# vniclas/VFM-Registration

Measured on AMD Instinct MI355X. Metric: registrations/sec (20k<->200k pts, 384-D), higher is better.
Workload: dtype fp6 (MX e2m3) coarse pass (scaled MFMA, fp32 scores + bounds from measured residuals) + int8 rescan (exact integer scores) + f32 refinement + f64 exact decision / f64 RANSAC

## Files before the change

### vfm-registration_amd/csrc/config.cpp

```cpp
#include "common.h"
#include "config.h"

#include <string.h>

#include <new>

struct vfm_config {
    VfmConfig c;
};

static const VfmConfig k_factory{};
static thread_local const VfmConfig* t_bound = nullptr;

const VfmConfig& vfm_cfg() { return t_bound ? *t_bound : k_factory; }

namespace {
struct Field {
    const char* name;
    int VfmConfig::*p;
};
const Field k_fields[] = {
    {"coarse_slices", &VfmConfig::force_slices},     {"match_stats", &VfmConfig::match_stats},
    {"i8_min_queries", &VfmConfig::i8_min_queries},  {"prep_grid", &VfmConfig::prep_grid},
    {"ransac_exact_only", &VfmConfig::ransac_exact_only}, {"ransac_fused", &VfmConfig::ransac_fused},
    {"coarse_qsets", &VfmConfig::coarse_qsets},      {"seed_units", &VfmConfig::seed_units},
    {"select_variant", &VfmConfig::select_variant},  {"mx6_t4", &VfmConfig::mx6_t4},
    {"mx6_tune", &VfmConfig::mx6_tune},
    {"mx6_ns3", &VfmConfig::mx6_ns3},                {"prep_form", &VfmConfig::prep_stream},
    {"finish_short", &VfmConfig::finish_short},      {"rescan_rows", &VfmConfig::rescan_rows},
    {"half_noi8", &VfmConfig::half_noi8},
    {"vit_preprocess_patch", &VfmConfig::vit_preprocess_patch}, {"vit_xcd", &VfmConfig::vit_xcd},
    {"vit_cfg_narrow", &VfmConfig::vit_cfg_narrow},  {"vit_cfg_wide", &VfmConfig::vit_cfg_wide},
    {"vit_wpw", &VfmConfig::vit_wpw},                {"vit_hot_a", &VfmConfig::vit_hot_a},
    {"vit_wide_tile", &VfmConfig::vit_wide_tile},    {"vit_lds_shape", &VfmConfig::vit_lds_shape},
    {"vit_att_lds_min", &VfmConfig::vit_att_lds_min}, {"vit_lds_min_wg", &VfmConfig::vit_lds_min_wg},
    {"vit_astat_min", &VfmConfig::vit_astat_min},    {"vit_astat_two", &VfmConfig::vit_astat_two},
    {"vit_astat_nw", &VfmConfig::vit_astat_nw},      {"vit_fused_qkv", &VfmConfig::vit_fused_qkv},
    {"vit_trace_fused", &VfmConfig::vit_trace_fused},  {"vit_fused_mlp", &VfmConfig::vit_fused_mlp},
    {"voxel_replay2", &VfmConfig::voxel_replay2},    {"voxel_one_launch", &VfmConfig::voxel_small},
    {"voxel_trace", &VfmConfig::voxel_trace},        {"voxel_grid_ppt", &VfmConfig::voxel_grid_ppt},
};

void set_coarse_variant(VfmConfig& c, int v) {
    if (v == 60 || v == 61) { c.rescan_rows = v == 61 ? 1 : 0; return; }
    if (v == 50 || v == 51) { c.finish_short = v == 51 ? 1 : 0; return; }
    if (v >= 40 && v <= 44) { c.prep_stream = v == 44 ? 4 : v == 43 ? 3 : v == 41 ? 1 : 0; return; }
    if (v == 32 || v == 33) { c.mx6_ns3 = v == 33 ? 1 : 0; return; }
    if (v == 30 || v == 31) { c.mx6_t4 = v == 30 ? 1 : 0; return; }
    c.seed_units = v == 7 ? 0 : 1;
    if (v == 7) v = 0;
    c.select_variant = v == 20 ? 1 : (v == 21 ? 2 : 0);
    if (v == 20 || v == 21) v = 0;
    c.coarse_qsets = v;
}
void set_vit_gemm(VfmConfig& c, int narrow, int wide) {
    switch (narrow) {
        case -3: case -4: c.vit_xcd = narrow == -3 ? 1 : 0; return;
        case -5: c.vit_lds_min_wg = wide; return;
        case -6: c.vit_lds_shape = wide; return;
        case -7: c.vit_att_lds_min = wide; return;
        case -8: c.vit_wpw = wide; return;
        case -9: c.vit_astat_min = wide; return;
        case -10: c.vit_astat_nw = wide; return;
        case -11: case -12: {
            unsigned long long v = (unsigned long long)(uintptr_t)c.vit_astat_dbg;
            v = narrow == -11 ? ((v & 0xffffffff00000000ull) | (unsigned)wide) : ((v & 0xffffffffull) | ((unsigned long long)(unsigned)wide << 32));
            c.vit_astat_dbg = reinterpret_cast<unsigned long long*>((uintptr_t)v);
            return;
        }
        case -14: c.vit_preprocess_patch = wide; return;
        case -15: c.vit_astat_two = wide; return;
        case -16: c.vit_hot_a = wide; return;
        case -17: c.vit_wide_tile = wide; return;
        default:
            c.vit_cfg_narrow = narrow ? narrow : 108;
            c.vit_cfg_wide = wide ? wide : 108;
    }
}
void set_voxel_small(VfmConfig& c, int on) {
    if (on == 2 || on == 3) c.voxel_replay2 = on == 3;
    else if (on >= 10 && on <= 10 + 64) c.voxel_grid_ppt = on - 10;
    else if (on == 100 || on == 101) c.voxel_trace = on - 100;
    else c.voxel_small = on;
}
}

VFM_EXPORT int vfm_config_create(vfm_config_t** out) {
    VFM_CHECK_ARG(out, "config_create: null pointer");
    *out = new (std::nothrow) vfm_config();
    if (!*out) return vfm_fail(VFM_EINVAL, "config_create: out of memory");
    return VFM_OK;
}
VFM_EXPORT int vfm_config_destroy(vfm_config_t* cfg) {
    if (cfg && t_bound == &cfg->c) t_bound = nullptr;
    delete cfg;
    return VFM_OK;
}
VFM_EXPORT int vfm_config_use(const vfm_config_t* cfg) {
    t_bound = cfg ? &cfg->c : nullptr;
    return VFM_OK;
}
VFM_EXPORT int vfm_config_set(vfm_config_t* cfg, const char* key, int64_t value) {
    VFM_CHECK_ARG(cfg && key, "config_set: null pointer");
    if ((!strcmp(key, "coarse_variant") && value == 42) || (!strcmp(key, "prep_form") && value == 2))
        return vfm_fail(VFM_EINVAL, "config_set: %s %lld (fp6 operand preparation by width) has been removed", key, (long long)value);
    if (!strcmp(key, "coarse_variant")) { set_coarse_variant(cfg->c, (int)value); return VFM_OK; }
    if (!strcmp(key, "voxel_small")) { set_voxel_small(cfg->c, (int)value); return VFM_OK; }
    if (!strcmp(key, "vit_gemm")) { set_vit_gemm(cfg->c, (int)(value >> 32), (int)(int32_t)(uint32_t)(value & 0xffffffffll)); return VFM_OK; }
    for (const Field& f : k_fields)
        if (!strcmp(key, f.name)) {
            cfg->c.*(f.p) = (int)value;
            return VFM_OK;
        }
    return vfm_fail(VFM_EINVAL, "config_set: unknown key '%s'", key);
}
VFM_EXPORT int vfm_config_get(const vfm_config_t* cfg, const char* key, int64_t* value) {
    VFM_CHECK_ARG(key && value, "config_get: null pointer");
    const VfmConfig& c = cfg ? cfg->c : vfm_cfg();
    for (const Field& f : k_fields)
        if (!strcmp(key, f.name)) {
            *value = c.*(f.p);
            return VFM_OK;
        }
    return vfm_fail(VFM_EINVAL, "config_get: unknown key '%s'", key);
}
```

### vfm-registration_amd/csrc/config.h

```cpp
#pragma once

struct VfmConfig {
    int force_slices = 0;
    int coarse_qsets = 0;
    int seed_units = 1;
    int select_variant = 0;
    int mx6_t4 = 1;
    int mx6_ns3 = 1;
    int prep_stream = 3;
    int finish_short = 0;
    int half_noi8 = 1;
    int rescan_rows = 1;
    int mx6_tune = 0;
    int match_stats = 0;
    int i8_min_queries = 0;
    int prep_grid = -1;
    int ransac_exact_only = 0;
    int ransac_fused = 2;
    int vit_preprocess_patch = 1, vit_xcd = 1, vit_cfg_narrow = 108, vit_cfg_wide = 108, vit_wpw = 0, vit_hot_a = 0, vit_wide_tile = 0,
        vit_lds_shape = 23, vit_att_lds_min = 1, vit_lds_min_wg = 256, vit_astat_min = 0, vit_astat_two = 1, vit_astat_nw = 0,
        vit_trace_fused = 0,
        vit_fused_mlp = 0,
        vit_fused_qkv = 0;
    unsigned long long* vit_astat_dbg = nullptr;
    int voxel_replay2 = 1, voxel_small = 1, voxel_trace = 0, voxel_grid_ppt = 0;
};

const VfmConfig& vfm_cfg();
```

### vfm-registration_amd/csrc/match_finish.hip

```cpp
#include "match_internal.h"

namespace vfmm {
namespace {

constexpr int SELECT_GROUPS = 16;
__global__ __launch_bounds__(64 * SELECT_GROUPS) void match_select_kernel(const uint2* __restrict__ partials, int nchunks, int npad,
                                                           int64_t n, int first_pad_chunk,
                                                           const unsigned* __restrict__ qmax,
                                                           const float* __restrict__ invq, float window,
                                                           I8Bounds ib, float gate, int chunk_lds, int* __restrict__ cand_cnt,
                                                           unsigned* __restrict__ cand, int cap, int* __restrict__ fb_count,
                                                           int* __restrict__ fb_list, int stats) {
    extern __shared__ __attribute__((aligned(16))) unsigned char select_smem[];
    __shared__ int lcnt[64];
    __shared__ int lresc[64];
    __shared__ unsigned lub[64];
    const int qq = threadIdx.x & 63, g = threadIdx.x >> 6;
    const int64_t q = (int64_t)blockIdx.x * 64 + qq;
    if (g == 0) {
        lcnt[qq] = 0;
        lresc[qq] = 0;
        lub[qq] = 0u;
    }
    float2* lchunk = reinterpret_cast<float2*>(select_smem);
// ... 1258 lines not shown
__global__ __launch_bounds__(256) void match_rescan_kernel(int64_t n, int64_t m, int d, I8Bounds ib, const uint4* __restrict__ q8,
                                                           const uint4* __restrict__ b8, const unsigned* __restrict__ qmax,
                                                           int* __restrict__ cand_cnt, unsigned* __restrict__ cand, int cap,
                                                           unsigned* __restrict__ hits, int hcap, int* __restrict__ fb_count,
                                                           int* __restrict__ fb_list, int use_gate, float gate,
                                                           const int* __restrict__ guard, L2Terms l2) {
    __shared__ uint4 l_q8[4][48];
    const int lane = lane_id(), wave = threadIdx.x >> 6;
    const int64_t qi = (int64_t)blockIdx.x * 4 + wave;
    if (qi >= n) return;
    if (guard && *guard) {
        if (lane == 0) cand_cnt[qi] = 0;
        return;
    }
    const int cnt = cand_cnt[qi];
    if (cnt <= 0) return;
    if (cnt > cap) {
        if (lane == 0) {
            cand_cnt[qi] = -1;
            fb_list[atomicAdd(fb_count, 1)] = (int)qi;
        }
        return;
    }
    unsigned* mycand = cand + (size_t)qi * cap;
    unsigned* myhits = hits + (size_t)qi * hcap;
    const int units8 = d >> 4;
    if (lane < units8) l_q8[wave][lane] = q8[(size_t)(qi >> 5) * (units8 * 32) + (size_t)lane * 32 + (qi & 31)];
    const float eq = ib.qerr[qi];
    const float sq = ib.qstep[qi >> 7], A = eq * 1.0001220703125f + 1.0e-6f, mult = 1.0001220703125f + eq;
    const float qlow = use_gate ? gate : key_float(qmax[qi]);
    const float qn_l2 = l2.qn ? l2.qn[qi] : 0.0f;
    __builtin_amdgcn_wave_barrier();
    int nhit = 0;
    const bool direct = cnt <= 64;
    unsigned* out = direct ? mycand : myhits;
    const int ocap = direct ? cap : hcap;
    for (int e0 = 0; e0 < cnt; e0 += 64) {
        const unsigned batch = (e0 + lane < cnt) ? mycand[e0 + lane] : 0u;
        const int nb = cnt - e0 < 64 ? cnt - e0 : 64;
        for (int j = 0; j < nb; ++j) {
            const unsigned entry = __shfl(batch, j);
            const int c = (int)(entry >> 8);
            if (!(entry & 128u)) {
                if (lane == 0 && nhit < ocap) out[nhit] = entry;
                ++nhit;
                continue;
            }
            const long long base = (long long)c * CHUNK_ROWS;
            const float sc = sq * ib.bstep[c], bound = A + mult * ib.berr[c];
            const uint4* src0 = b8 + ((size_t)c * 4 + (lane >> 5)) * (size_t)(units8 * 32) + (lane & 31);
            const uint4* src1 = src0 + 2 * (size_t)(units8 * 32);
            int acc2[2] = {0, 0};
            for (int u0 = 0; u0 < units8; u0 += 8) {
                uint4 bv0[8], bv1[8];
#pragma unroll
                for (int k = 0; k < 8; ++k) {
                    bv0[k] = src0[(u0 + k) * 32];
                    bv1[k] = src1[(u0 + k) * 32];
                }
#pragma unroll
                for (int k = 0; k < 8; ++k) {
                    const uint4 qv = l_q8[wave][u0 + k];
                    acc2[0] = __builtin_amdgcn_sdot4((int)bv0[k].x, (int)qv.x, acc2[0], false);
                    acc2[0] = __builtin_amdgcn_sdot4((int)bv0[k].y, (int)qv.y, acc2[0], false);
                    acc2[0] = __builtin_amdgcn_sdot4((int)bv0[k].z, (int)qv.z, acc2[0], false);
                    acc2[0] = __builtin_amdgcn_sdot4((int)bv0[k].w, (int)qv.w, acc2[0], false);
                    acc2[1] = __builtin_amdgcn_sdot4((int)bv1[k].x, (int)qv.x, acc2[1], false);
                    acc2[1] = __builtin_amdgcn_sdot4((int)bv1[k].y, (int)qv.y, acc2[1], false);
                    acc2[1] = __builtin_amdgcn_sdot4((int)bv1[k].z, (int)qv.z, acc2[1], false);
                    acc2[1] = __builtin_amdgcn_sdot4((int)bv1[k].w, (int)qv.w, acc2[1], false);
                }
            }
#pragma unroll
            for (int half = 0; half < 2; ++half) {
                const int rr = lane + 64 * half;
                const int acc = acc2[half];
                float up = sc * (float)acc + bound;
                if (l2.qn) up = l2_upper_row(qn_l2, l2.bn[base + rr], up, l2.slack);
                const bool hit = base + rr < m && up >= qlow;
                const unsigned long long bal = __ballot(hit);
                if (hit) {
                    const int pos = nhit + __popcll(bal & ((1ull << lane) - 1ull));
                    if (pos < ocap) out[pos] = ((unsigned)c << 8) | (unsigned)rr;
                }
                nhit += __popcll(bal);
            }
        }
    }
    if (nhit > ocap || nhit > cap) {
        if (lane == 0) {
            cand_cnt[qi] = -1;
            const int slot = atomicAdd(fb_count, 1);
            fb_list[slot] = (int)qi;
        }
        return;
    }
    if (!direct) {
        __builtin_amdgcn_fence(__ATOMIC_SEQ_CST, "agent");
        for (int i = lane; i < nhit; i += 64) mycand[i] = myhits[i];
    }
    if (lane == 0) {
        cand_cnt[qi] = nhit;
    }
}

template <int NT>
__global__ __launch_bounds__(256) void match_refine_kernel(Rows q, const float* __restrict__ invq,
                                                           Rows b, const float* __restrict__ invb,
                                                           int64_t n, int64_t m, int d, float w2, int* __restrict__ cand_cnt,
                                                           unsigned* __restrict__ cand, int cap, int* __restrict__ fb_count,
                                                           int* __restrict__ fb_list, int stats, const int* __restrict__ todo,
                                                           const int* __restrict__ todo_count, const float* __restrict__ cand_up,
                                                           const unsigned* __restrict__ hit_cnt, I8Bounds ib) {
    __shared__ unsigned l_row[4][REFINE_KEEP];
    __shared__ float l_sc[4][REFINE_KEEP];
    const int lane = lane_id(), wave = threadIdx.x >> 6;
    const int64_t slot0 = (int64_t)blockIdx.x * 4 + wave;
    const int64_t nslots = todo ? (int64_t)*todo_count : n;
  for (int64_t slot = slot0; slot < nslots; slot += (int64_t)gridDim.x * 4) {
    const int64_t qi = todo ? (int64_t)todo[slot] : slot;
    if (qi >= n) return;
    unsigned* mycand = cand + (size_t)qi * cap;
    const float* myup = cand_up ? cand_up + (size_t)qi * cap : nullptr;
    const int cnt = cand_cnt[qi];
    const int hits = cand_up ? (int)hit_cnt[(size_t)qi * BIN_CNT_STRIDE] : 0;
    const float eq = cand_up ? ib.qerr[qi] : 0.0f;
    const float iq = invq[qi];
    const unsigned ce0 = mycand[lane];
    const float up0 = cand_up ? myup[lane] : 0.0f;
    if (cnt <= 0) continue;
    bool flagged = lane < cnt && (ce0 & 128u) != 0u;
    for (int e = 64 + lane; e < cnt; e += 64) flagged |= (mycand[e] & 128u) != 0u;
    if (cnt < REFINE_MIN && !__any(flagged)) continue;
    RefineWave<NT> R;
    R.init(q, iq, qi, b, invb, d, w2, l_row[wave], l_sc[wave]);
    int split = cnt;
    float lowest = -__builtin_inff();
    if (cand_up) {
        split = cnt - hits < 0 ? 0 : cnt - hits;
        const float A = eq * 1.0001220703125f + 1.0e-6f, mult = 1.0001220703125f + eq;
        if (lane >= split && lane < cnt) {
            const float bnd = A + mult * ib.berr[ce0 >> 8];
            if (up0 < 3.0e38f) lowest = (up0 - 2.0f * bnd) - 4.0e-6f;
        }
        for (int e = (split > 64 ? split : 64) + lane; e < cnt; e += 64) {
            const float u = myup[e];
            const float bnd = A + mult * ib.berr[mycand[e] >> 8];
            if (u < 3.0e38f) lowest = fmaxf(lowest, (u - 2.0f * bnd) - 4.0e-6f);
        }
#pragma unroll
        for (int off = 32; off >= 1; off >>= 1) lowest = fmaxf(lowest, __shfl_xor(lowest, off));
    }
    for (int e0 = 0; e0 < cnt; e0 += 64) {
        const int nblk = cnt - e0 < 64 ? cnt - e0 : 64;
        long long myrow = -1;
        if (lane < nblk) {
            const unsigned ce = e0 == 0 ? ce0 : mycand[e0 + lane];
            if (!(ce & 128u)) {
                myrow = (long long)(ce >> 8) * CHUNK_ROWS + (ce & 127u);
                if (myrow >= m) myrow = -1;
                if (e0 + lane >= split && (e0 == 0 ? up0 : myup[e0 + lane]) < lowest) myrow = -1;
            }
        }
        if (!__any(myrow >= 0)) continue;
        const unsigned long long keep = __ballot(myrow >= 0);
        const int nkeep = __popcll(keep);
        {
            int need = lane, src = 0;
            unsigned long long rest = keep;
#pragma unroll
            for (int sh = 32; sh >= 1; sh >>= 1) {
                const unsigned long long lowmask = (1ull << sh) - 1ull;
                const int below = __popcll(rest & lowmask);
                if (need >= below) {
                    need -= below;
                    rest >>= sh;
                    src += sh;
                } else {
                    rest &= lowmask;
                }
            }
            const long long packed = __shfl(myrow, src & 63);
            myrow = lane < nkeep ? packed : -1;
        }
        const int nblk_keep = nkeep;
        auto row_at = [&](int p) { return p < nblk_keep ? __shfl(myrow, (p + R.g) & 63) : -1ll; };
        typename RefineWave<NT>::Row ra, rb;
        long long rowa = row_at(0), rowb;
        R.load4(ra, rowa);
        for (int p = 0; p < nblk_keep; p += 8) {
            rowb = row_at(p + 4);
            R.load4(rb, rowb);
            if (__any(rowa >= 0)) R.consider(rowa, R.dot4(ra, rowa));
            rowa = row_at(p + 8);
            R.load4(ra, rowa);
            if (__any(rowb >= 0)) R.consider(rowb, R.dot4(rb, rowb));
        }
    }
    for (int e = 0; e < cnt; ++e) {
        const unsigned ce = mycand[e];
        if (!(ce & 128u)) continue;
        const long long base = (long long)(ce >> 8) * CHUNK_ROWS;
        for (int r0 = 0; r0 < CHUNK_ROWS; r0 += 4) {
            long long row = base + r0 + R.g;
            if (row >= m) row = -1;
            if (__any(row >= 0)) R.consider(row, R.score4(row));
        }
    }
    if (R.overflow) continue;
    R.finish(qi, mycand, cand_cnt, fb_count, fb_list, stats);
    __builtin_amdgcn_wave_barrier();
  }
}

__global__ __launch_bounds__(256) void match_filter_refine_kernel(Rows q, const float* __restrict__ invq,
                                                                  Rows b, const float* __restrict__ invb,
                                                                  int64_t n, int64_t m, int d, float window, float w2,
                                                                  const unsigned* __restrict__ qmax,
                                                                  const unsigned* __restrict__ rec_cnt, const uint2* __restrict__ rec,
                                                                  int rcap, int* __restrict__ cand_cnt, unsigned* __restrict__ cand,
                                                                  int cap, int* __restrict__ fb_count, int* __restrict__ fb_list, int stats) {
    __shared__ unsigned l_row[4][REFINE_KEEP];
    __shared__ float l_sc[4][REFINE_KEEP];
    __shared__ unsigned l_cand[4][FILTER_LDS_ROWS];
    const int lane = lane_id(), wave = threadIdx.x >> 6;
    const int64_t qi = (int64_t)blockIdx.x * 4 + wave;
    if (qi >= n) return;
    unsigned* mycand = cand + (size_t)qi * cap;
    const float iq = invq[qi];
    if (iq == 0.0f) {
        if (lane == 0) cand_cnt[qi] = 0;
        return;
    }
    const unsigned total = rec_cnt[qi];
    if (stats && lane == 0) {
        atomicAdd(fb_count + 4, (int)total);
    }
    if (total > (unsigned)rcap || m <= 0) {
        if (lane == 0) {
            cand_cnt[qi] = -1;
            const int slot = atomicAdd(fb_count, 1);
            fb_list[slot] = (int)qi;
        }
        return;
    }
    const unsigned thr = __float_as_uint(__uint_as_float(qmax[qi]) - window);
    const uint2* myrec = rec + (size_t)qi * rcap;
    unsigned* lc = l_cand[wave];
    int ncand = 0;
    for (unsigned e0 = 0; e0 < total; e0 += 64) {
        const unsigned e = e0 + lane;
        uint2 r = make_uint2(0u, 0u);
        if (e < total) r = myrec[e];
        const bool in = e < total && r.y >= thr;
        const unsigned long long bal = __ballot(in);
        if (in) lc[ncand + __popcll(bal & ((1ull << lane) - 1ull))] = r.x;
        ncand += __popcll(bal);
    }
    __builtin_amdgcn_wave_barrier();
    if (stats && lane == 0) {
        atomicAdd(fb_count + 2, ncand);
        int bin = 0;
        while ((1 << bin) < ncand && bin < 15) ++bin;
        atomicAdd(fb_count + 8 + bin, 1);
    }
    if (ncand < REFINE_MIN) {
        if (lane < ncand) {
            const unsigned row = lc[lane];
            mycand[lane] = ((row / CHUNK_ROWS) << 8) | (row % CHUNK_ROWS);
        }
        if (lane == 0) cand_cnt[qi] = ncand;
        return;
    }
    RefineWave<12> R;
    R.init(q, iq, qi, b, invb, d, w2, l_row[wave], l_sc[wave]);
    for (int e0 = 0; e0 < ncand; e0 += 4) {
        const long long row = (e0 + R.g < ncand) ? (long long)lc[e0 + R.g] : -1;
        R.consider(row, R.score4(row));
    }
    if (R.overflow && ncand <= cap) {
        for (int e = lane; e < ncand; e += 64) {
            const unsigned row = lc[e];
            mycand[e] = ((row / CHUNK_ROWS) << 8) | (row % CHUNK_ROWS);
        }
        if (lane == 0) cand_cnt[qi] = ncand;
        return;
    }
    R.finish(qi, mycand, cand_cnt, fb_count, fb_list, stats);
}

__device__ __forceinline__ double dot_norm_f64(const float* __restrict__ qrow_n, Rows b, int64_t brow, float invb, int d) {
    double acc = 0.0;
    for (int k = 0; k < d; k += 4) {
        const float4 bv = b.ld4(brow + k);
        const float b0 = bv.x * invb, b1 = bv.y * invb, b2 = bv.z * invb, b3 = bv.w * invb;
        acc = acc + (double)qrow_n[k + 0] * (double)b0;
        acc = acc + (double)qrow_n[k + 1] * (double)b1;
        acc = acc + (double)qrow_n[k + 2] * (double)b2;
        acc = acc + (double)qrow_n[k + 3] * (double)b3;
    }
    return acc;
}

constexpr int RS_KC = 96;
constexpr int RS_STRIDE = RS_KC + 1;
constexpr int RS_PAIRS = 1024;
__global__ __launch_bounds__(256) void match_rescore_kernel(Rows q, const float* __restrict__ invq,
                                                            Rows b, const float* __restrict__ invb,
                                                            int64_t n, int64_t m, int d, const int* __restrict__ cand_cnt,
                                                            const unsigned* __restrict__ cand, int cap,
                                                            int64_t* __restrict__ idx_out, float* __restrict__ sim_out, float min_sim) {
    extern __shared__ __attribute__((aligned(16))) unsigned char smem[];
    double* P = reinterpret_cast<double*>(smem);
    double* pscore = P + 64 * RS_STRIDE;
    float* qn = reinterpret_cast<float*>(pscore + RS_PAIRS);
    __shared__ unsigned p_j[RS_PAIRS];
    __shared__ unsigned char p_q[RS_PAIRS];
    __shared__ long long s_j[64];
    __shared__ float s_iq[64], s_ib[64];
    __shared__ int s_ql[64];
    __shared__ int s_total;
    const int lane = lane_id(), wave = threadIdx.x >> 6;
    const int64_t q0 = (int64_t)blockIdx.x * 64;
    const int64_t qi = q0 + lane;
    const bool owner = wave == 0;
    const bool have = owner && qi < n;
    const float iq = have ? invq[qi] : 0.0f;
    int cnt = have ? cand_cnt[qi] : 0;
    if (iq == 0.0f || cnt < 0) cnt = 0;
    bool any_rescan = false;
    int my_off = 0, my_pairs = 0;
    const unsigned* mycand = cand + (size_t)(have ? qi : 0) * cap;
    auto row_of = [&](unsigned ce) { return (long long)(ce >> 8) * CHUNK_ROWS + (ce & 127u); };
    if (owner) {
        for (int e = 0; e < cnt; ++e) {
            const unsigned ce = mycand[e];
            if (ce & 128u) any_rescan = true;
            else if (row_of(ce) < m) ++my_pairs;
        }
        int incl = my_pairs;
#pragma unroll
        for (int off = 1; off < 64; off <<= 1) {
            const int v = __shfl_up(incl, off);
            if (lane >= off) incl += v;
        }
        my_off = incl - my_pairs;
        if (lane == 63) s_total = incl;
    }
    __syncthreads();
    const int total = s_total;
    double best = 0.0;
    long long bj = -1;
    for (int E0 = 0; E0 < total; E0 += RS_PAIRS) {
        const int ecount = min(RS_PAIRS, total - E0);
        if (owner) {
            int k = my_off;
            for (int e = 0; e < cnt; ++e) {
                const unsigned ce = mycand[e];
                if ((ce & 128u) || row_of(ce) >= m) continue;
                if (k >= E0 && k < E0 + RS_PAIRS) {
                    p_j[k - E0] = (unsigned)row_of(ce);
                    p_q[k - E0] = (unsigned char)lane;
                }
                ++k;
            }
        }
        __syncthreads();
        for (int p0 = 0; p0 < ecount; p0 += 64) {
            long long j = -1;
            if (owner) {
                const int pid = p0 + lane;
                const int ql = (pid < ecount) ? (int)p_q[pid] : 0;
                const float iqq = __shfl(iq, ql);
                float ibb = 0.f;
                if (pid < ecount) {
                    j = (long long)p_j[pid];
                    ibb = invb[j];
                }
                s_j[lane] = j;
                s_ql[lane] = ql;
                s_iq[lane] = iqq;
                s_ib[lane] = ibb;
            }
            __syncthreads();
            double acc = 0.0;
            const int sub = lane >> 5, l4 = lane & 31;
            float4 qv[8], bv[8];
            auto fetch = [&](int k0) {
                const int kn = min(RS_KC, d - k0);
#pragma unroll
                for (int it = 0; it < 8; ++it) {
                    const int sl = 16 * wave + 2 * it + sub;
                    const long long jj = s_j[sl];
                    if (jj >= 0 && 4 * l4 < kn) {
                        qv[it] = q.ld4((q0 + s_ql[sl]) * (int64_t)d + k0 + 4 * l4);
                        bv[it] = b.ld4(jj * (int64_t)d + k0 + 4 * l4);
                    }
                }
            };
            fetch(0);
            for (int k0 = 0; k0 < d; k0 += RS_KC) {
                const int kn = min(RS_KC, d - k0);
#pragma unroll
                for (int it = 0; it < 8; ++it) {
                    const int sl = 16 * wave + 2 * it + sub;
                    if (s_j[sl] >= 0 && 4 * l4 < kn) {
                        const float iqq = s_iq[sl], ibb = s_ib[sl];
                        double* dst = P + sl * RS_STRIDE + 4 * l4;
                        dst[0] = (double)(qv[it].x * iqq) * (double)(bv[it].x * ibb);
                        dst[1] = (double)(qv[it].y * iqq) * (double)(bv[it].y * ibb);
                        dst[2] = (double)(qv[it].z * iqq) * (double)(bv[it].z * ibb);
                        dst[3] = (double)(qv[it].w * iqq) * (double)(bv[it].w * ibb);
                    }
                }
                __syncthreads();
                if (k0 + RS_KC < d) fetch(k0 + RS_KC);
                if (owner && j >= 0) {
                    const double* src = P + lane * RS_STRIDE;
                    int k = 0;
                    for (; k + 8 <= kn; k += 8) {
                        double v[8];
#pragma unroll
                        for (int u = 0; u < 8; ++u) v[u] = src[k + u];
#pragma unroll
                        for (int u = 0; u < 8; ++u) acc = acc + v[u];
                    }
                    for (; k < kn; ++k) acc = acc + src[k];
                }
                __syncthreads();
            }
            if (owner && j >= 0) pscore[p0 + lane] = acc;
        }
        __syncthreads();
        if (owner) {
            const int lo = max(my_off, E0), hi = min(my_off + my_pairs, E0 + RS_PAIRS);
            for (int k = lo; k < hi; ++k) {
                const long long j = (long long)p_j[k - E0];
                const double sc = pscore[k - E0];
                if (bj < 0 || sc > best || (sc == best && j < bj)) {
                    best = sc;
                    bj = j;
                }
            }
        }
        __syncthreads();
    }
    if (!owner) return;
    if (__any(any_rescan)) {
        for (int ql = 0; ql < 64; ++ql) {
            if (!__shfl((int)any_rescan, ql)) continue;
            const int64_t qq = q0 + ql;
            const float iqq = __shfl(iq, ql);
            const int cq = __shfl(cnt, ql);
            __builtin_amdgcn_wave_barrier();
            for (int k = lane * 4; k < d; k += 256) {
                float4 v = q.ld4(qq * (int64_t)d + k);
                v.x = v.x * iqq; v.y = v.y * iqq; v.z = v.z * iqq; v.w = v.w * iqq;
                *reinterpret_cast<float4*>(qn + k) = v;
            }
            __builtin_amdgcn_wave_barrier();
            double rbest = 0.0;
            long long rj = -1;
            for (int e = 0; e < cq; ++e) {
                const unsigned ce = cand[(size_t)qq * cap + e];
                if (!(ce & 128u)) continue;
                const long long base = (long long)(ce >> 8) * CHUNK_ROWS;
                for (int li = lane; li < CHUNK_ROWS; li += 64) {
                    const long long j = base + li;
                    if (j < m) {
                        const double sc = dot_norm_f64(qn, b, j * (int64_t)d, invb[j], d);
                        if (rj < 0 || sc > rbest || (sc == rbest && j < rj)) {
                            rbest = sc;
                            rj = j;
                        }
                    }
                }
            }
            wave_argmax(rbest, rj);
            if (lane == ql && rj >= 0 && (bj < 0 || rbest > best || (rbest == best && rj < bj))) {
                best = rbest;
                bj = rj;
            }
        }
    }
    if (!have) return;
    if (iq == 0.0f) {
        idx_out[qi] = (m > 0) ? 0 : -1;
        sim_out[qi] = 0.0f;
    } else if (cand_cnt[qi] >= 0) {
        const bool ok = !((float)best < min_sim) && bj >= 0;
        idx_out[qi] = ok ? bj : -1;
        sim_out[qi] = ok ? (float)best : -2.0f;
    } else if (cand_cnt[qi] == -2) {
        idx_out[qi] = -1;
        sim_out[qi] = -2.0f;
    }
}

__global__ __launch_bounds__(256) void match_exact_kernel(Rows q, const float* __restrict__ invq,
                                                          Rows b, const float* __restrict__ invb,
                                                          int64_t n, int64_t m, int d, const int* __restrict__ list,
                                                          const int* __restrict__ list_count,
                                                          int64_t* __restrict__ idx_out, float* __restrict__ sim_out) {
    extern __shared__ __attribute__((aligned(16))) unsigned char smem[];
    float* qn = reinterpret_cast<float*>(smem);
    double* rs = reinterpret_cast<double*>(smem + (((size_t)d * 4 + 15) & ~(size_t)15));
    long long* rj = reinterpret_cast<long long*>(rs + 4);
    const int64_t count = list ? (int64_t)*list_count : n;
    for (int64_t e = blockIdx.x; e < count; e += gridDim.x) {
        const int64_t qi = list ? (int64_t)list[e] : e;
        const float iq = invq ? invq[qi] : 1.0f;
        __syncthreads();
        for (int k = threadIdx.x; k < d; k += 256) qn[k] = q.ld1(qi * (int64_t)d + k) * iq;
        __syncthreads();
        double best = 0.0;
        long long bj = -1;
        for (long long j = threadIdx.x; j < m; j += 256) {
            const double s = dot_norm_f64(qn, b, j * (int64_t)d, invb ? invb[j] : 1.0f, d);
            if (bj < 0 || s > best) {
                best = s;
                bj = j;
            }
        }
        wave_argmax(best, bj);
        if (lane_id() == 0) {
            rs[threadIdx.x >> 6] = best;
            rj[threadIdx.x >> 6] = bj;
        }
        __syncthreads();
        if (threadIdx.x == 0) {
            for (int w = 1; w < 4; ++w)
                if (rj[w] >= 0 && (rj[0] < 0 || rs[w] > rs[0] || (rs[w] == rs[0] && rj[w] < rj[0]))) {
                    rs[0] = rs[w];
                    rj[0] = rj[w];
                }
            idx_out[qi] = (m > 0) ? rj[0] : -1;
            sim_out[qi] = (m > 0) ? (float)rs[0] : 0.0f;
        }
    }
}

constexpr int TC_ITERS = 4;
__global__ __launch_bounds__(1024) void threshold_compact_kernel(const float* __restrict__ sim, const int64_t* __restrict__ idx,
                                                                 int64_t n, double thr, int64_t* __restrict__ keep,
                                                                 int64_t* __restrict__ count, int32_t* __restrict__ corres,
                                                                 const double* __restrict__ qxyz, const double* __restrict__ bxyz,
                                                                 double* __restrict__ src_out, double* __restrict__ tgt_out) {
    __shared__ int wsum[TC_ITERS][16];
    const int lane = lane_id(), wave = threadIdx.x >> 6;
    int64_t base = 0;
    for (int64_t s0 = 0; s0 < n; s0 += (int64_t)TC_ITERS * 1024) {
        bool valid[TC_ITERS];
        int before[TC_ITERS];
        float sv[TC_ITERS];
#pragma unroll
        for (int t = 0; t < TC_ITERS; ++t) {
            const int64_t i = s0 + (int64_t)t * 1024 + threadIdx.x;
            sv[t] = i < n ? sim[i] : 0.0f;
        }
#pragma unroll
        for (int t = 0; t < TC_ITERS; ++t) {
            const int64_t i = s0 + (int64_t)t * 1024 + threadIdx.x;
            valid[t] = (i < n) && !((double)sv[t] < thr);
            const unsigned long long bal = __ballot(valid[t]);
            before[t] = __popcll(bal & ((1ull << lane) - 1ull));
            if (lane == 0) wsum[t][wave] = __popcll(bal);
        }
        __syncthreads();
        int64_t k[TC_ITERS];
        int j[TC_ITERS];
        int64_t run = base;
#pragma unroll
        for (int t = 0; t < TC_ITERS; ++t) {
            int woff = 0, tot = 0;
#pragma unroll
            for (int w = 0; w < 16; ++w) {
                const int c = wsum[t][w];
                if (w < wave) woff += c;
                tot += c;
            }
            k[t] = run + woff + before[t];
            run += tot;
            const int64_t i = s0 + (int64_t)t * 1024 + threadIdx.x;
            j[t] = (valid[t] && idx) ? (int)idx[i] : 0;
        }
        base = run;
#pragma unroll
        for (int t = 0; t < TC_ITERS; ++t) {
            if (!valid[t]) continue;
            const int64_t i = s0 + (int64_t)t * 1024 + threadIdx.x;
            keep[k[t]] = i;
            if (corres) {
                corres[2 * k[t] + 0] = (int32_t)i;
                corres[2 * k[t] + 1] = (int32_t)j[t];
            }
            if (src_out) {
                src_out[3 * k[t] + 0] = qxyz[3 * i + 0];
                src_out[3 * k[t] + 1] = qxyz[3 * i + 1];
                src_out[3 * k[t] + 2] = qxyz[3 * i + 2];
            }
            if (tgt_out) {
                tgt_out[3 * k[t] + 0] = bxyz[3 * (int64_t)j[t] + 0];
                tgt_out[3 * k[t] + 1] = bxyz[3 * (int64_t)j[t] + 1];
                tgt_out[3 * k[t] + 2] = bxyz[3 * (int64_t)j[t] + 2];
            }
        }
        __syncthreads();
    }
    if (threadIdx.x == 0) *count = base;
}

__global__ __launch_bounds__(256) void inv_norm_kernel(const float* __restrict__ x, int64_t rows, int d,
                                                       float* __restrict__ inv_out) {
    const int64_t r = (int64_t)blockIdx.x * 4 + (threadIdx.x >> 6);
    if (r >= rows) return;
    float4 v[4];
    float nr = row_sumsq_wave(x + r * (int64_t)d, d, v);
    float inv = inv_norm_from_sumsq(nr);
    if (lane_id() == 0) inv_out[r] = (nr > 0.0f) ? inv : 1.0f;
}

}

int do_search_finish(Rows q, const void* qprep, int64_t n, Rows b, const void* bprep, int64_t m, int d,
                     int64_t* idx_out, float* sim_out, void* ws, hipStream_t st, bool gated, float gate, int records) {
    SearchPlan plan;
    VFM_TRY(resolve_search(plan, records, d, n, m, gated, true));
    VFM_TRY(check_plan_gate(plan.gate_test, gate, "search_finish"));
    Prepared Q = carve_prepared(const_cast<void*>(qprep), n, d);
    Prepared B = carve_prepared(const_cast<void*>(bprep), m, d);
    SearchWs w = carve_search(ws, n, m);
    const CoarseArgs a = coarse_args(Q, B, w, n, m, coarse_qblock(d));
    const float w2 = 2.0f * (float)(d / 16 + 4 + 2) * 5.9604645e-8f;
    const bool i8 = plan.quantised(), half = plan.gate_test, use_bins = plan.use_bins;
    const I8Bounds sel_ib = plan_bounds(plan, Q, B), ib = i8_bounds(Q, B, i8, plan.top2 ? 1 : 0);
    const int chunk_lds = i8 && (size_t)a.nchunks * sizeof(float2) <= 63 * 1024;
    const int* guard = half ? w.fb_count + HALF_GUARD_FLAG : (const int*)nullptr;
    for (int i = 0; i < plan.nsteps; ++i) {
        const FinishStep step = plan.steps[i];
        switch (step) {
            case FIN_FILTER_REFINE:
                hipLaunchKernelGGL(match_filter_refine_kernel, dim3((unsigned)((n + 3) / 4)), dim3(256), 0, st, q, Q.inv, b, B.inv, n, m, d,
                                   DEFAULT_WINDOW, w2, w.qmax, w.rec_cnt, w.rec, w.rcap, w.cand_cnt, w.cand, w.cap, w.fb_count, w.fb_list, vfm_cfg().match_stats);
                break;
            case FIN_PILOT_BIN:
                hipLaunchKernelGGL(match_pilot_bin_kernel, dim3((unsigned)((n + 255) / 256)), dim3(256), 0, st, n, (const unsigned long long*)w.qbest,
                                   (const float*)Q.inv, w.bin_cnt, w.bins, w.bin_cap, a.nchunks);
                break;
            case FIN_PILOT_RESCAN:
                VFM_TRY(launch_rescan_chunk(w, a.nchunks, n, m, d, i8_bounds(Q, B, true, VFM_RECORDS_BEST), Q, B, 0, gate, (const int*)nullptr,
                                            L2Terms{nullptr, nullptr, 0.0f}, st, true));
                VFM_CHECK_HIP(hipMemsetAsync(w.bin_cnt, 0, (size_t)((a.nchunks + 63) / 64 * 64) * BIN_CNT_STRIDE * sizeof(unsigned), st));
                break;
            case FIN_BIN_SURVIVORS:
                hipLaunchKernelGGL(match_bin_survivors_kernel, dim3(256), dim3(256), 0, st, reinterpret_cast<const unsigned*>(w.partials),
                                   mx6_survivor_slot_words(), (const int*)w.fb_count, w.bin_cnt, w.bins, w.bin_cap, w.cand_cnt, w.cand, w.cap);
                break;
            case FIN_SELECT_HALF: {
                const int half_lds = (size_t)a.nchunks * 12 <= 63 * 1024;
                hipLaunchKernelGGL(match_select_half_kernel, dim3((unsigned)a.nq_tiles), dim3(64 * 8), half_lds ? (size_t)a.nchunks * 12 : 0,
                                   st, reinterpret_cast<const unsigned*>(w.partials), a.nchunks, n, Q.inv, sel_ib, (const float*)Q.rest,
                                   (const float*)B.grest, gate, half_lds, w.cand_cnt, w.cand, w.cap, w.fb_count, w.fb_list, vfm_cfg().match_stats,
                                   use_bins ? w.bin_cnt : (unsigned*)nullptr, use_bins ? w.bins : (int*)nullptr, w.bin_cap);
                break;
            }
            case FIN_SELECT_TOP2:
                hipLaunchKernelGGL(match_select_top2_kernel, dim3((unsigned)a.nq_tiles), dim3(64 * SELECT_TOP2_WAVES),
                                   chunk_lds ? (size_t)a.nchunks * sizeof(float2) : 0, st, (const uint2*)w.partials, a.nchunks, n, a.first_pad_chunk,
                                   (const unsigned*)w.qmax, Q.inv, sel_ib, gate, chunk_lds, w.cand_cnt, w.cand, w.cap, w.fb_count, w.fb_list, vfm_cfg().match_stats);
                break;
            case FIN_SELECT_BEST: {
                const int best_lds = chunk_lds && use_bins && (size_t)a.nchunks * 12 <= 63 * 1024 && a.nchunks < 65536 ? 2 : chunk_lds;
                hipLaunchKernelGGL(match_select_best_kernel, dim3((unsigned)a.nq_tiles), dim3(64 * SELECT_BEST_WAVES),
                                   best_lds == 2 ? (size_t)a.nchunks * 12 : chunk_lds ? (size_t)a.nchunks * sizeof(float2) : 0, st,
                                   reinterpret_cast<const unsigned*>(w.partials), a.nchunks, n, (const unsigned*)w.qmax, Q.inv, sel_ib, gate, best_lds,
                                   w.cand_cnt, w.cand, w.cap, w.fb_count, w.fb_list, vfm_cfg().match_stats, use_bins ? w.bin_cnt : (unsigned*)nullptr,
                                   use_bins ? w.bins : (int*)nullptr, a.first_pad_chunk, w.bin_cap);
                break;
            }
            case FIN_SELECT:
                hipLaunchKernelGGL(match_select_kernel, dim3((unsigned)((n + 63) / 64)), dim3(64 * SELECT_GROUPS),
                                   chunk_lds ? (size_t)a.nchunks * sizeof(float2) : 0, st, w.partials, a.nchunks, a.npad, n, a.first_pad_chunk, w.qmax,
                                   Q.inv, DEFAULT_WINDOW, sel_ib, gate, chunk_lds, w.cand_cnt, w.cand, w.cap, w.fb_count, w.fb_list, vfm_cfg().match_stats);
                break;
            case FIN_HALF_GUARD:
                hipLaunchKernelGGL(half_guard_kernel, dim3(1), dim3(256), 0, st, w.fb_count, (const unsigned*)w.bin_cnt, a.nchunks,
                                   plan.fused ? 1 : 0, (long long)HALF_GUARD_PER_QUERY * (long long)n);
                break;
            case FIN_GUARD_FALLBACK:
                hipLaunchKernelGGL(match_guard_fallback_kernel, dim3((unsigned)((n + 255) / 256)), dim3(256), 0, st, n, (const float*)Q.inv, guard,
                                   w.cand_cnt, w.fb_count, w.fb_list);
                break;
            case FIN_RESCAN:
                hipLaunchKernelGGL(match_rescan_kernel, dim3((unsigned)((n + 3) / 4)), dim3(256), 0, st, n, m, d, ib,
                                   (const uint4*)Q.tiles8, (const uint4*)B.tiles8, (const unsigned*)w.qmax, w.cand_cnt, w.cand, w.cap,
                                   reinterpret_cast<unsigned*>(w.rec), 2 * w.rcap, w.fb_count, w.fb_list, half ? 1 : 0, gate, guard,
                                   L2Terms{nullptr, nullptr, 0.0f});
                break;
            case FIN_GATEPASS:
#define VFM_GATEPASS(KS)                                                                                                        \
    hipLaunchKernelGGL(match_gatepass_kernel<KS>, dim3((unsigned)a.nchunks), dim3(256), 0, st, n, m, a.nq_tiles, ib, (const float*)Q.inv, \
                       (const uint4*)Q.tiles8, (const uint4*)B.tiles8, gate, w.cand_cnt, w.cand, w.cap, guard, w.qmax)
                switch (d / 32) {
                    case 8: VFM_GATEPASS(8); break;
                    case 12: VFM_GATEPASS(12); break;
                    case 16: VFM_GATEPASS(16); break;
                    case 20: VFM_GATEPASS(20); break;
                    default: VFM_GATEPASS(24); break;
                }
#undef VFM_GATEPASS
                break;
            case FIN_RESCAN_CHUNK:
                VFM_TRY(launch_rescan_chunk(w, a.nchunks, n, m, d, ib, Q, B, half ? 1 : 0, gate, guard, L2Terms{nullptr, nullptr, 0.0f}, st));
                break;
            case FIN_RESCAN_CHUNK_MX6H:
                VFM_TRY(d == 384 ? launch_rescan_chunk_mx6h<3>(w, a.nchunks, n, m, Q, B, gate, guard, st)
                                 : launch_rescan_chunk_mx6h<2>(w, a.nchunks, n, m, Q, B, gate, guard, st));
                break;
            case FIN_RESCAN_CLOSE:
                hipLaunchKernelGGL(match_rescan_close_kernel, dim3((unsigned)((n + 255) / 256)), dim3(256), 0, st, n, w.cand_cnt, w.cap,
                                   w.fb_count, w.fb_list, reinterpret_cast<int*>(w.rec_cnt), half ? (const float*)Q.inv : (const float*)nullptr,
                                   (const unsigned*)w.hit_cnt);
                break;
            case FIN_REFINE: {
                const unsigned grid = (unsigned)((n + 3) / 4);
#define VFM_REFINE(NT)                                                                                                          \
    hipLaunchKernelGGL(match_refine_kernel<NT>, dim3(grid), dim3(256), 0, st, q, Q.inv, b, B.inv, n, m, d, w2, w.cand_cnt, w.cand, \
                       w.cap, w.fb_count, w.fb_list, vfm_cfg().match_stats, i8 ? (const int*)w.rec_cnt : (const int*)nullptr,      \
                       i8 ? (const int*)(w.fb_count + 6) : (const int*)nullptr, use_bins ? (const float*)w.cand_up : (const float*)nullptr, \
                       i8 ? (const unsigned*)w.hit_cnt : (const unsigned*)nullptr, ib)
                if (!i8 || d > 512) VFM_REFINE(12);
                else if (d <= 256) VFM_REFINE(4);
                else if (d <= 384) VFM_REFINE(6);
                else VFM_REFINE(8);
#undef VFM_REFINE
                break;
            }
            case FIN_RESCORE: {
                const size_t lds = (size_t)(64 * RS_STRIDE + RS_PAIRS) * sizeof(double) + (size_t)d * sizeof(float);
                static unsigned long long attr_set = 0ull;
                if (!attr_done(attr_set)) {
                    VFM_CHECK_HIP(hipFuncSetAttribute(reinterpret_cast<const void*>(&match_rescore_kernel),
                                                      hipFuncAttributeMaxDynamicSharedMemorySize, 96 * 1024));
                    attr_mark(attr_set);
                }
                hipLaunchKernelGGL(match_rescore_kernel, dim3((unsigned)((n + 63) / 64)), dim3(256), lds, st, q, Q.inv, b, B.inv, n, m,
                                   d, w.cand_cnt, w.cand, w.cap, idx_out, sim_out, half ? gate : -__builtin_inff());
                break;
            }
            case FIN_EXACT:
                hipLaunchKernelGGL(match_exact_kernel, dim3(256), dim3(256), (((size_t)d * 4 + 15) & ~(size_t)15) + 64, st, q, Q.inv,
                                   b, B.inv, n, m, d, w.fb_list, w.fb_count, idx_out, sim_out);
                break;
        }
        VFM_CHECK_LAUNCH(finish_step_name(step));
    }
    return VFM_OK;
}

int launch_i8_rescans(const SearchWs& w, const CoarseArgs& a, const Prepared& Q, const Prepared& B, int64_t n, int64_t m, int d,
                      bool use_bins, L2Terms l2, hipStream_t st) {
    const I8Bounds ib = i8_bounds(Q, B, true, VFM_RECORDS_BEST);
    hipLaunchKernelGGL(match_rescan_kernel, dim3((unsigned)((n + 3) / 4)), dim3(256), 0, st, n, m, d, ib, (const uint4*)Q.tiles8,
                       (const uint4*)B.tiles8, (const unsigned*)w.qmax, w.cand_cnt, w.cand, w.cap, reinterpret_cast<unsigned*>(w.rec),
                       2 * w.rcap, w.fb_count, w.fb_list, 0, 0.0f, (const int*)nullptr, l2);
    VFM_CHECK_LAUNCH("match_rescan_kernel");
    if (use_bins) {
        const int rc = launch_rescan_chunk(w, a.nchunks, n, m, d, ib, Q, B, 0, 0.0f, (const int*)nullptr, l2, st);
        if (rc != VFM_OK) return rc;
    }
    hipLaunchKernelGGL(match_rescan_close_kernel, dim3((unsigned)((n + 255) / 256)), dim3(256), 0, st, n, w.cand_cnt, w.cap, w.fb_count,
                       w.fb_list, reinterpret_cast<int*>(w.rec_cnt), (const float*)nullptr, (const unsigned*)w.hit_cnt);
    VFM_CHECK_LAUNCH("match_rescan_close_kernel");
    return VFM_OK;
}

int probe_half_select(const SearchPlan& plan, const void* qprep, int64_t n, const void* bprep, int64_t m, int d, void* ws, float gate, hipStream_t st) {
    Prepared Q = carve_prepared(const_cast<void*>(qprep), n, d);
    Prepared B = carve_prepared(const_cast<void*>(bprep), m, d);
    SearchWs w = carve_search(ws, n, m);
    const CoarseArgs a = coarse_args(Q, B, w, n, m, coarse_qblock(d));
    const int half_lds = (size_t)a.nchunks * 12 <= 63 * 1024;
    hipLaunchKernelGGL(match_select_half_kernel, dim3((unsigned)a.nq_tiles), dim3(64 * 8), half_lds ? (size_t)a.nchunks * 12 : 0, st,
                       reinterpret_cast<const unsigned*>(w.partials), a.nchunks, n, Q.inv, plan_bounds(plan, Q, B),
                       (const float*)Q.rest, (const float*)B.grest, gate, half_lds, w.cand_cnt, (unsigned*)nullptr, w.cap, w.fb_count,
                       w.fb_list, 0, (unsigned*)nullptr, (int*)nullptr, w.bin_cap);
    VFM_CHECK_LAUNCH("match_select_half_kernel(probe)");
    return VFM_OK;
}

int launch_select_dense(const SearchWs& w, const CoarseArgs& a, const float* qinv, int64_t n, hipStream_t st) {
    hipLaunchKernelGGL(match_select_kernel, dim3((unsigned)((n + 63) / 64)), dim3(64 * SELECT_GROUPS), 0, st, w.partials, a.nchunks,
                       a.npad, n, a.first_pad_chunk, w.qmax, qinv, DEFAULT_WINDOW, i8_bounds(Prepared{}, Prepared{}, false),
                       -__builtin_inff(), 0, w.cand_cnt, w.cand, w.cap, w.fb_count, w.fb_list, vfm_cfg().match_stats);
    VFM_CHECK_LAUNCH("match_select_kernel");
    return VFM_OK;
}

int exact_ip_top1(const float* q, int64_t n, const float* b, int64_t m, int d, int64_t* idx_out, float* sim_out, void* ws,
                  hipStream_t st) {
    VfmCarver c(ws);
    float* invq = c.take<float>((size_t)n);
    float* invb = c.take<float>((size_t)m);
    hipLaunchKernelGGL(inv_norm_kernel, dim3((unsigned)((n + 3) / 4)), dim3(256), 0, st, q, n, d, invq);
    hipLaunchKernelGGL(inv_norm_kernel, dim3((unsigned)((m + 3) / 4)), dim3(256), 0, st, b, m, d, invb);
    VFM_CHECK_LAUNCH("inv_norm_kernel");
    const unsigned grid = (unsigned)(n < 4096 ? n : 4096);
    hipLaunchKernelGGL(match_exact_kernel, dim3(grid), dim3(256), (((size_t)d * 4 + 15) & ~(size_t)15) + 64, st, q,
                       invq, b, invb, n, m, d, (const int*)nullptr, (const int*)nullptr, idx_out, sim_out);
    VFM_CHECK_LAUNCH("match_exact_kernel");
    return VFM_OK;
}

}

using namespace vfmm;

VFM_EXPORT int vfm_threshold_compact(const float* sim, const int64_t* idx, int64_t n, double thr, int64_t* keep_out,
                                     int64_t* count_out, int32_t* corres_out, const double* q_xyz, const double* b_xyz,
                                     double* src_xyz_out, double* tgt_xyz_out, vfm_stream_t stream) {
    VFM_CHECK_ARG(n >= 0 && sim && keep_out && count_out, "threshold_compact: bad arguments");
    VFM_CHECK_ARG(!(corres_out || tgt_xyz_out) || idx, "threshold_compact: idx required for corres / tgt output");
    VFM_CHECK_ARG(!src_xyz_out || q_xyz, "threshold_compact: q_xyz required");
    VFM_CHECK_ARG(!tgt_xyz_out || b_xyz, "threshold_compact: b_xyz required");
    hipLaunchKernelGGL(threshold_compact_kernel, dim3(1), dim3(1024), 0, (hipStream_t)stream, sim, idx, n, thr, keep_out,
                       count_out, corres_out, q_xyz, b_xyz, src_xyz_out, tgt_xyz_out);
    VFM_CHECK_LAUNCH("threshold_compact_kernel");
    return VFM_OK;
}
```

Baseline: 2123.

## Let rescore workgroups own 256 queries with per-thread f64 pair dots

Adds a templated variant of the rescore kernel in which all four waves own queries (256 per workgroup). In this variant each thread computes a whole f64 query-candidate dot product from global memory with double-buffered float4 loads, replacing the cooperative LDS-staged tile path. Wave prefix sums are combined across waves. The variant is selected by default when the plan is in half mode, otherwise through a new config key. It aims to cut idle waves and LDS barrier traffic, but each thread now does long serial dot products with no LDS reuse, and there are fewer workgroups.

```diff
diff --git a/vfm-registration_amd/csrc/config.cpp b/vfm-registration_amd/csrc/config.cpp
--- a/vfm-registration_amd/csrc/config.cpp
+++ b/vfm-registration_amd/csrc/config.cpp
@@ -28,7 +28,7 @@
     {"mx6_tune", &VfmConfig::mx6_tune},
     {"mx6_ns3", &VfmConfig::mx6_ns3},                {"prep_form", &VfmConfig::prep_stream},
     {"finish_short", &VfmConfig::finish_short},      {"rescan_rows", &VfmConfig::rescan_rows},
-    {"half_noi8", &VfmConfig::half_noi8},
+    {"half_noi8", &VfmConfig::half_noi8},            {"rescore_block", &VfmConfig::rescore_block},
     {"vit_preprocess_patch", &VfmConfig::vit_preprocess_patch}, {"vit_xcd", &VfmConfig::vit_xcd},
     {"vit_cfg_narrow", &VfmConfig::vit_cfg_narrow},  {"vit_cfg_wide", &VfmConfig::vit_cfg_wide},
     {"vit_wpw", &VfmConfig::vit_wpw},                {"vit_hot_a", &VfmConfig::vit_hot_a},
@@ -104,6 +104,8 @@
     VFM_CHECK_ARG(cfg && key, "config_set: null pointer");
     if ((!strcmp(key, "coarse_variant") && value == 42) || (!strcmp(key, "prep_form") && value == 2))
         return vfm_fail(VFM_EINVAL, "config_set: %s %lld (fp6 operand preparation by width) has been removed", key, (long long)value);
+    if (!strcmp(key, "rescore_block") && value != 64 && value != 256)
+        return vfm_fail(VFM_EINVAL, "config_set: rescore_block %lld (a workgroup of match_rescore_kernel owns 64 or 256 queries)", (long long)value);
     if (!strcmp(key, "coarse_variant")) { set_coarse_variant(cfg->c, (int)value); return VFM_OK; }
     if (!strcmp(key, "voxel_small")) { set_voxel_small(cfg->c, (int)value); return VFM_OK; }
     if (!strcmp(key, "vit_gemm")) { set_vit_gemm(cfg->c, (int)(value >> 32), (int)(int32_t)(uint32_t)(value & 0xffffffffll)); return VFM_OK; }
diff --git a/vfm-registration_amd/csrc/config.h b/vfm-registration_amd/csrc/config.h
--- a/vfm-registration_amd/csrc/config.h
+++ b/vfm-registration_amd/csrc/config.h
@@ -10,6 +10,7 @@
     int prep_stream = 3;
     int finish_short = 0;
     int half_noi8 = 1;
+    int rescore_block = 0;
     int rescan_rows = 1;
     int mx6_tune = 0;
     int match_stats = 0;
diff --git a/vfm-registration_amd/csrc/match_finish.hip b/vfm-registration_amd/csrc/match_finish.hip
--- a/vfm-registration_amd/csrc/match_finish.hip
+++ b/vfm-registration_amd/csrc/match_finish.hip
@@ -1584,9 +1584,42 @@
     return acc;
 }
 
+__device__ __forceinline__ double dot_pair_f64(Rows q, int64_t qe, float iq, Rows b, int64_t be, float ib, int d) {
+    double acc = 0.0;
+    auto add4 = [&](const float4& qv, const float4& bv) __attribute__((always_inline)) {
+        acc = acc + (double)(qv.x * iq) * (double)(bv.x * ib);
+        acc = acc + (double)(qv.y * iq) * (double)(bv.y * ib);
+        acc = acc + (double)(qv.z * iq) * (double)(bv.z * ib);
+        acc = acc + (double)(qv.w * iq) * (double)(bv.w * ib);
+    };
+    float4 q0[8], b0[8], q1[8], b1[8];
+    auto fetch = [&](float4 (&qq)[8], float4 (&bb)[8], int k) __attribute__((always_inline)) {
+#pragma unroll
+        for (int i = 0; i < 8; ++i) {
+            qq[i] = q.ld4(qe + k + 4 * i);
+            bb[i] = b.ld4(be + k + 4 * i);
+        }
+    };
+    auto use = [&](const float4 (&qq)[8], const float4 (&bb)[8]) __attribute__((always_inline)) {
+#pragma unroll
+        for (int i = 0; i < 8; ++i) add4(qq[i], bb[i]);
+    };
+    const int dmain = d & ~63;
+    if (dmain) fetch(q0, b0, 0);
+    for (int k = 0; k < dmain; k += 64) {
+        fetch(q1, b1, k + 32);
+        use(q0, b0);
+        if (k + 64 < dmain) fetch(q0, b0, k + 64);
+        use(q1, b1);
+    }
+    for (int k = dmain; k < d; k += 4) add4(q.ld4(qe + k), b.ld4(be + k));
+    return acc;
+}
+
 constexpr int RS_KC = 96;
 constexpr int RS_STRIDE = RS_KC + 1;
 constexpr int RS_PAIRS = 1024;
+template <int QB>
 __global__ __launch_bounds__(256) void match_rescore_kernel(Rows q, const float* __restrict__ invq,
                                                             Rows b, const float* __restrict__ invb,
                                                             int64_t n, int64_t m, int d, const int* __restrict__ cand_cnt,
@@ -1594,18 +1627,22 @@
                                                             int64_t* __restrict__ idx_out, float* __restrict__ sim_out, float min_sim) {
     extern __shared__ __attribute__((aligned(16))) unsigned char smem[];
     double* P = reinterpret_cast<double*>(smem);
-    double* pscore = P + 64 * RS_STRIDE;
+    double* pscore = P + (QB > 64 ? 0 : 64 * RS_STRIDE);
     float* qn = reinterpret_cast<float*>(pscore + RS_PAIRS);
+    constexpr int NW = QB / 64;
+    static_assert(QB == 64 || QB == 256, "a workgroup's queries: wave 0's lanes, or its 256 threads (p_q holds a query as a byte)");
     __shared__ unsigned p_j[RS_PAIRS];
     __shared__ unsigned char p_q[RS_PAIRS];
-    __shared__ long long s_j[64];
-    __shared__ float s_iq[64], s_ib[64];
-    __shared__ int s_ql[64];
-    __shared__ int s_total;
+    __shared__ long long s_j[QB > 64 ? 1 : 64];
+    __shared__ float s_iq[QB > 64 ? 1 : 64], s_ib[QB > 64 ? 1 : 64];
+    __shared__ int s_ql[QB > 64 ? 1 : 64];
+    __shared__ int s_wsum[4];
+    __shared__ float s_qinv[QB > 64 ? QB : 1];
     const int lane = lane_id(), wave = threadIdx.x >> 6;
-    const int64_t q0 = (int64_t)blockIdx.x * 64;
-    const int64_t qi = q0 + lane;
-    const bool owner = wave == 0;
+    const int64_t q0 = (int64_t)blockIdx.x * QB;
+    const int myq = QB > 64 ? (int)threadIdx.x : lane;
+    const int64_t qi = q0 + myq;
+    const bool owner = wave < NW, lead = wave == 0;
     const bool have = owner && qi < n;
     const float iq = have ? invq[qi] : 0.0f;
     int cnt = have ? cand_cnt[qi] : 0;
@@ -1627,10 +1664,17 @@
             if (lane >= off) incl += v;
         }
         my_off = incl - my_pairs;
-        if (lane == 63) s_total = incl;
+        if (lane == 63) s_wsum[wave] = incl;
+        if constexpr (QB > 64) s_qinv[myq] = iq;
     }
     __syncthreads();
-    const int total = s_total;
+    int total = 0;
+#pragma unroll
+    for (int w = 0; w < NW; ++w) {
+        const int ws = s_wsum[w];
+        if (w < wave) my_off += ws;
+        total += ws;
+    }
     double best = 0.0;
     long long bj = -1;
     for (int E0 = 0; E0 < total; E0 += RS_PAIRS) {
@@ -1642,15 +1686,26 @@
                 if ((ce & 128u) || row_of(ce) >= m) continue;
                 if (k >= E0 && k < E0 + RS_PAIRS) {
                     p_j[k - E0] = (unsigned)row_of(ce);
-                    p_q[k - E0] = (unsigned char)lane;
+                    p_q[k - E0] = (unsigned char)myq;
                 }
                 ++k;
             }
         }
         __syncthreads();
+        if constexpr (QB > 64) {
+            const int per = (ecount + 3) >> 2, wend = min(ecount, (wave + 1) * per);
+            for (int p0 = wave * per; p0 < wend; p0 += 64) {
+                const int pid = p0 + lane;
+                if (pid < wend) {
+                    const long long j = (long long)p_j[pid];
+                    const int ql = (int)p_q[pid];
+                    pscore[pid] = dot_pair_f64(q, (q0 + ql) * (int64_t)d, s_qinv[ql], b, j * (int64_t)d, invb[j], d);
+                }
+            }
+        } else {
         for (int p0 = 0; p0 < ecount; p0 += 64) {
             long long j = -1;
-            if (owner) {
+            if (lead) {
                 const int pid = p0 + lane;
                 const int ql = (pid < ecount) ? (int)p_q[pid] : 0;
                 const float iqq = __shfl(iq, ql);
@@ -1697,7 +1752,7 @@
                 }
                 __syncthreads();
                 if (k0 + RS_KC < d) fetch(k0 + RS_KC);
-                if (owner && j >= 0) {
+                if (lead && j >= 0) {
                     const double* src = P + lane * RS_STRIDE;
                     int k = 0;
                     for (; k + 8 <= kn; k += 8) {
@@ -1711,7 +1766,8 @@
                 }
                 __syncthreads();
             }
-            if (owner && j >= 0) pscore[p0 + lane] = acc;
+            if (lead && j >= 0) pscore[p0 + lane] = acc;
+        }
         }
         __syncthreads();
         if (owner) {
@@ -1729,9 +1785,10 @@
     }
     if (!owner) return;
     if (__any(any_rescan)) {
+        if constexpr (QB > 64) qn += (size_t)wave * d;
         for (int ql = 0; ql < 64; ++ql) {
             if (!__shfl((int)any_rescan, ql)) continue;
-            const int64_t qq = q0 + ql;
+            const int64_t qq = q0 + (myq - lane) + ql;
             const float iqq = __shfl(iq, ql);
             const int cq = __shfl(cnt, ql);
             __builtin_amdgcn_wave_barrier();
@@ -1900,6 +1957,21 @@
     float nr = row_sumsq_wave(x + r * (int64_t)d, d, v);
     float inv = inv_norm_from_sumsq(nr);
     if (lane_id() == 0) inv_out[r] = (nr > 0.0f) ? inv : 1.0f;
+}
+
+template <int QB>
+int launch_rescore(Rows q, const Prepared& Q, Rows b, const Prepared& B, int64_t n, int64_t m, int d, const SearchWs& w,
+                   int64_t* idx_out, float* sim_out, float min_sim, hipStream_t st) {
+    const size_t lds = (size_t)((QB > 64 ? 0 : 64 * RS_STRIDE) + RS_PAIRS) * sizeof(double) + (size_t)(QB / 64) * d * sizeof(float);
+    static unsigned long long attr_set = 0ull;
+    if (!attr_done(attr_set)) {
+        VFM_CHECK_HIP(hipFuncSetAttribute(reinterpret_cast<const void*>(&match_rescore_kernel<QB>),
+                                          hipFuncAttributeMaxDynamicSharedMemorySize, 96 * 1024));
+        attr_mark(attr_set);
+    }
+    hipLaunchKernelGGL(match_rescore_kernel<QB>, dim3((unsigned)((n + QB - 1) / QB)), dim3(256), lds, st, q, Q.inv, b, B.inv, n, m, d,
+                       w.cand_cnt, w.cand, w.cap, idx_out, sim_out, min_sim);
+    return VFM_OK;
 }
 
 }
@@ -2018,18 +2090,11 @@
 #undef VFM_REFINE
                 break;
             }
-            case FIN_RESCORE: {
-                const size_t lds = (size_t)(64 * RS_STRIDE + RS_PAIRS) * sizeof(double) + (size_t)d * sizeof(float);
-                static unsigned long long attr_set = 0ull;
-                if (!attr_done(attr_set)) {
-                    VFM_CHECK_HIP(hipFuncSetAttribute(reinterpret_cast<const void*>(&match_rescore_kernel),
-                                                      hipFuncAttributeMaxDynamicSharedMemorySize, 96 * 1024));
-                    attr_mark(attr_set);
-                }
-                hipLaunchKernelGGL(match_rescore_kernel, dim3((unsigned)((n + 63) / 64)), dim3(256), lds, st, q, Q.inv, b, B.inv, n, m,
-                                   d, w.cand_cnt, w.cand, w.cap, idx_out, sim_out, half ? gate : -__builtin_inff());
+            case FIN_RESCORE:
+                VFM_TRY((vfm_cfg().rescore_block ? vfm_cfg().rescore_block : plan.half ? 256 : 64) == 256
+                            ? launch_rescore<256>(q, Q, b, B, n, m, d, w, idx_out, sim_out, half ? gate : -__builtin_inff(), st)
+                            : launch_rescore<64>(q, Q, b, B, n, m, d, w, idx_out, sim_out, half ? gate : -__builtin_inff(), st));
                 break;
-            }
             case FIN_EXACT:
                 hipLaunchKernelGGL(match_exact_kernel, dim3(256), dim3(256), (((size_t)d * 4 + 15) & ~(size_t)15) + 64, st, q, Q.inv,
                                    b, B.inv, n, m, d, w.fb_list, w.fb_count, idx_out, sim_out);
```

Measured after the change: 2172, median of 6. +2.3%, better.
